# harmoniqs/DirectTrajOpt.jl

Hardware: AMD Instinct MI355X
Metric: knot-points/sec for eval_constraint_jacobian, 256-state×2000-knot bilinear (higher is better)
Workload: dtype f64; 1 GPU; configs[2]: 256-state bilinear, 4 drives, N=2000 knots per GPU (make_scaled_problem shape, Philox seed 42), callback=jacobian; state_dim=256, drives=4, knots_per_gpu=2000, knots_total=2000, parallelism=knot-range shards x1, outputs_finite=True, max_squarings=1, sweep_terms=25

## Files before the change

directtrajopt.jl_amd/csrc/dto_engine.cpp:

```cpp
#include "../../include/dto_engine.h"

#include <hip/hip_runtime.h>

#include <algorithm>
#include <chrono>
#include <cmath>
#include <cstdio>
#include <cstdlib>
#include <cstring>
#include <functional>
#include <limits>
#include <map>
#include <string>
#include <vector>

#include "dto_comm.h"
#include "dto_hostxfer.h"
#include "dto_kernels.h"

#include <memory>

using namespace dto;

namespace {
// ... 31 lines not shown

struct SweepWork {
    double* slab = nullptr;
    unsigned* arrive = nullptr;
    size_t cap = 0;
    int counters = 0;
};

struct BilHost {
    KBil k;
    SweepBuf fw{}, ad{};
    int T_alloc = 0;
    std::vector<double> g1;
    std::vector<double> n2;
    double* d_g1 = nullptr;
    double* d_n2 = nullptr;
    ChainWork chain{};
    int chain_cap = 0;
    unsigned long long* d_hump = nullptr;
    double hump_logH[4] = {0, 0, 0, 0};
    int hump_kend[4] = {0, 0, 0, 0};
    bool hump_valid = false;
    int cache_kind = 0, cache_steps = 0;
    int plan_q = 0, plan_dub = 0;
    bool p_terms = false;
    int p_steps = 0;
    int p_nblk = 0;
    SweepWork cluster_work[2];
    SweepWork gs_work[2];
    bool small = false;
    double* d_Gs = nullptr;
    bool use_basis = false;
    BasisSet basis[3]{};
    BasisSet basis_all{};
    bool pairing = false;
    double* EP = nullptr;
    double* Upair = nullptr;
    double* d_Btab = nullptr;
};

struct ConHost {
    KCon k{};
    int equality = 0;
    int64_t n_times_total = 0;
    int64_t row_off = 0;
    std::vector<int64_t> times0;
    std::vector<int32_t> comps;
    int g_dim = 1;
    bool external = false;
    bool global = false;
    int ext_slot = -1;
    std::vector<double> jac0;
    std::vector<double> hess0;
    KExtTerm xk{};
};

struct ExtObjHost {
    double weight = 1.0;
    bool global = false;
    std::vector<int32_t> comps, gcomps;
    std::vector<int64_t> times0;
    KExtTerm k{};
    int ext_slot = -1;
};

struct ExtSlot {
    dto_external_values v{nullptr, nullptr, nullptr};
// ... 74 lines not shown
    double* d_out = nullptr;
    size_t d_out_cap = 0;
    double* d_partial = nullptr;
    double* d_f = nullptr;
    double* d_bounds = nullptr;
    int32_t* d_plan = nullptr;
    double* d_jac_scratch = nullptr;
    double* d_w = nullptr;
    int64_t* d_conbase = nullptr;
    int64_t* d_crow_ptr = nullptr;
    int64_t* d_crow_col = nullptr;
    int64_t* d_crow_pos = nullptr;
    int64_t* d_con_rows = nullptr;
    double* h_pinned = nullptr;
    bool smax_pending = false;
    hipStream_t stream = nullptr;
    hipStream_t stream2 = nullptr;
    hipStream_t stream_rb = nullptr;
    hipEvent_t ev_fork = nullptr, ev_join = nullptr, ev_stats = nullptr, ev_chain = nullptr, ev_rb = nullptr, ev_zero = nullptr;

    bool reuse = false;
    double* d_Zcache = nullptr;
    int32_t* d_eq = nullptr;
    bool profiling = false;
    std::vector<ProfRec> prof;
    int64_t sweep_forms[5] = {0, 0, 0, 0, 0};
    std::vector<hipEvent_t> ev_pool;
    int last_smax = 0, last_terms = 0;
    int expm_form = 0;
    int overlap_sweep = 1;
    int sweep_form = 0;
    int chain_form = 0;
    int n_cu = 256;
    int chain_chunk = 0;
    int deterministic = 0;
    hipEvent_t ev_done = nullptr;
    bool stats_pending = false;
    int32_t* h_stats = nullptr;
    int last_form = 0;
    std::unique_ptr<Comm> comm;
    int comm_rank = -1;
    std::vector<std::pair<int64_t, int64_t>> rank_ranges;
    GatherPlan gather_plan[4];
    std::vector<Slab> cons_segments;
    std::vector<int> cons_segment_root;
    int64_t* d_ranges = nullptr;
    double* hp_slab = nullptr;
    bool hp_slab_primed = false;
    bool hp_index = false;
    KHessProduct hp{};
    int64_t hp_nnz = 0;
    int64_t* d_hp_pos = nullptr;
    double* d_hp_val = nullptr;
    double* d_hp_Z = nullptr;
    double* d_hp_mu = nullptr;
    double* d_hp_v = nullptr;
    int32_t* d_hp_eq = nullptr;
    double hp_sigma = 0.0;
    bool hp_valid = false;
    uint64_t gen = 0, hp_gen = 0;
    double hp_setup_ms = 0.0;
    double hp_bytes = 0.0;
    std::vector<void*> owned;

    ~dto_handle();
};
// ... 477 lines not shown
        enum_multisets(m1, r, cur, 0, sets[r]);
        for (size_t a = 0; a < sets[r].size(); ++a) index[r][sets[r][a]] = (int)a;
    }
    double* tmp = own(h, dalloc<double>(nn));
    std::vector<double*> S(5, nullptr);
    S[1] = const_cast<double*>(b.k.G);
    for (int r = 2; r <= 4; ++r) {
        const int cnt = (int)sets[r].size(), cntpad = ((cnt + 15) / 16) * 16;
        S[r] = own(h, dalloc<double>(nn * cntpad));
        HIP_CHECK(hipMemsetAsync(S[r], 0, nn * cntpad * sizeof(double), h->stream));
        std::vector<int32_t> idx;
        for (int a = 0; a < cnt; ++a) {
            const std::vector<int>& al = sets[r][a];
            for (int v : al) idx.push_back(v);
            int last = -1;
            for (size_t p = 0; p < al.size(); ++p) {
                const int i = al[p];
                if (i == last) continue;
                last = i;
                std::vector<int> rest = al;
                rest.erase(rest.begin() + p);
                const double* prev = S[r - 1] + (size_t)index[r - 1][rest] * nn;
                launch_bgemm_plain(h->stream, npad, 1, b.k.G + (size_t)i * nn, prev, tmp);
                launch_add(h->stream, S[r] + (size_t)a * nn, tmp, (int64_t)nn);
            }
        }
        BasisSet& bs = b.basis[r - 2];
        bs.r = r; bs.cnt = cnt; bs.cntpad = cntpad; bs.S = S[r];
        bs.idx = own(h, dupload(idx));
        const int cappad = ((cap + 127) / 128) * 128;
        bs.coef = own(h, dalloc<double>((size_t)cappad * cntpad));
    }
    {
        int cnt = 1 + m1;
        for (int r = 2; r <= 4; ++r) cnt += (int)sets[r].size();
        const int cntpad = ((cnt + 15) / 16) * 16;
        double* Sall = own(h, dalloc<double>(nn * cntpad));
        HIP_CHECK(hipMemsetAsync(Sall, 0, nn * cntpad * sizeof(double), h->stream));
        std::vector<double> eye(nn, 0.0);
        for (int i = 0; i < b.k.n; ++i) eye[(size_t)i * npad + i] = 1.0;
        HIP_CHECK(hipMemcpyAsync(Sall, eye.data(), nn * sizeof(double), hipMemcpyHostToDevice, h->stream));
        HIP_CHECK(hipStreamSynchronize(h->stream));
        std::vector<int32_t> idx;
        size_t col = 1;
        for (int q = 0; q < 4; ++q) idx.push_back(-1);
        for (int r = 1; r <= 4; ++r) {
            HIP_CHECK(hipMemcpyAsync(Sall + col * nn, S[r], nn * sets[r].size() * sizeof(double), hipMemcpyDeviceToDevice, h->stream));
            col += sets[r].size();
            for (auto& al : sets[r]) {
                for (int q = 0; q < 4; ++q) idx.push_back(q < r ? al[q] : -1);
            }
        }
        BasisSet& bs = b.basis_all;
        bs.r = 4; bs.cnt = cnt; bs.cntpad = cntpad; bs.S = Sall;
        bs.idx = own(h, dupload(idx));
        const int cappad = ((cap + 127) / 128) * 128;
        bs.coef = own(h, dalloc<double>((size_t)cappad * cntpad));
    }
    HIP_CHECK(hipStreamSynchronize(h->stream));
    b.use_basis = true;
}

void alloc_chain(dto_handle* h, BilHost& b, int cap) {
    const size_t nn = (size_t)b.k.npad * b.k.npad;
    for (int i = 0; i < 9; ++i) b.chain.W[i] = own(h, dalloc<double>(nn * cap));
    b.chain.norms = own(h, dalloc<double>((size_t)cap * 4));
    b.chain.colsum = own(h, dalloc<double>((size_t)3 * cap * b.k.npad * (b.k.npad / 64)));
    if (!b.d_hump) b.d_hump = own(h, dalloc<unsigned long long>(8));
    b.chain.coef = own(h, dalloc<double>((size_t)cap * COEF_STRIDE));
    b.chain.s = own(h, dalloc<int32_t>(cap));
    b.chain.s3 = own(h, dalloc<int32_t>(cap));
    b.chain.smax = own(h, dalloc<int32_t>(8));
    HIP_CHECK(hipMemset(b.chain.smax, 0, 8 * sizeof(int32_t)));
    b.chain.d2max = reinterpret_cast<unsigned long long*>(b.chain.smax + 2);
    b.chain_cap = cap;
}

int chunk_size(const dto_handle* h, int npad) {
    const double budget = 40e9;
    int c = (int)(budget / (9.0 * npad * (double)npad * 8.0));
    c = std::max(8, (c / 8) * 8);
    return (int)std::min<int64_t>(c, std::max<int64_t>(h->P.n_int, 1));
}

double run_chain(dto_handle* h, BilHost& b, const double* dZ, double* vals, double b1max, hipStream_t st,
                 const std::function<void(double)>& after_last_enqueue = nullptr, const std::function<void()>& in_bubble = nullptr,
                 bool nothing_waits = false) {
    const int npad = b.k.npad;
    const int64_t nint = h->P.n_int;
    double d2max = 0.0;
// ... 15 lines not shown
        }
        if (nothing_waits) {
            HIP_CHECK(hipMemcpyAsync(h->h_pinned + 28, w.smax, sizeof(int32_t), hipMemcpyDeviceToHost, st));
            h->smax_pending = true;
            h->last_form = 0;
            if (in_bubble) in_bubble();
            if (h->on_chain_chunk) h->on_chain_chunk(0, (int)nint);
            if (after_last_enqueue) after_last_enqueue(0.0);
            return 0.0;
        }
        launch_hump(st, h->P, b.k, dZ, b.d_g1, h->P.kn_lo, (int)nint, w.norms, b.d_hump);
        int32_t* hs = reinterpret_cast<int32_t*>(h->h_pinned + 2);
        HIP_CHECK(hipMemcpyAsync(hs, w.smax, 8 * sizeof(int32_t), hipMemcpyDeviceToHost, st));
        HIP_CHECK(hipMemcpyAsync(h->h_pinned + 16, b.d_hump, 8 * sizeof(unsigned long long), hipMemcpyDeviceToHost, st));
        HIP_CHECK(hipEventRecord(h->ev_chain, st));
        if (in_bubble) in_bubble();
        HIP_CHECK(hipEventSynchronize(h->ev_chain));
        h->last_form = 0;
        h->last_smax = hs[0];
        read_hump(h, b);
        {
            double dv;
            memcpy(&dv, hs + 2, sizeof(double));
            d2max = dv;
        }
        if (h->on_chain_chunk) h->on_chain_chunk(0, (int)nint);
        if (after_last_enqueue) after_last_enqueue(d2max);
        return d2max;
    }
    const double gemm_flops = 2.0 * npad * (double)npad * npad;
    h->last_smax = 0;
    const int64_t nchunk = (nint + cap - 1) / cap;
    const int per = (int)std::min<int64_t>(cap, (((nint + nchunk - 1) / nchunk) + 7) / 8 * 8);
    for (int64_t c0 = 0; c0 < nint; c0 += per) {
        const int nb = (int)std::min<int64_t>(per, nint - c0);
        const int64_t int0 = h->P.kn_lo + c0;
        ChainWork& w = b.chain;
        const int nbpad = ((nb + 127) / 128) * 128;
        if (b.use_basis) {
            launch_fill(st, w.norms, (int64_t)nb * 4, INFINITY);
            double* outs[3] = {w.W[1], w.W[2], w.W[3]};
            const size_t cs_set = (size_t)cap * npad * (npad / 64);
            double* css[3] = {w.colsum, w.colsum + cs_set, w.colsum + 2 * cs_set};
            {
                ProfScope ps(h, st, CAT_BUILD_A, 8.0 * npad * (double)npad * nb);
                launch_build_A(st, h->P, b.k, dZ, int0, nb, w.W[0]);
            }
            launch_basis_coef_multi(st, h->P, b.k, 3, b.basis, dZ, int0, nb, nbpad);
            {
                const double cols = b.basis[0].cntpad + b.basis[1].cntpad + b.basis[2].cntpad;
                ProfScope ps(h, st, CAT_BASIS_MULTI, 2.0 * npad * (double)npad * cols * nb);
                launch_basis_gemm_multi(st, npad, nb, nbpad, 3, b.basis, outs, css);
            }
            launch_norm_from_colsum_multi(st, npad, nb, 3, css, w.norms);
        } else {
            {
                ProfScope ps(h, st, CAT_BUILD_A, 8.0 * npad * (double)npad * nb);
                launch_build_A(st, h->P, b.k, dZ, int0, nb, w.W[0]);
            }
            { ProfScope ps(h, st, CAT_BGEMM, gemm_flops * nb); launch_bgemm_plain(st, npad, nb, w.W[0], w.W[0], w.W[1]); }
            { ProfScope ps(h, st, CAT_BGEMM, gemm_flops * nb); launch_bgemm_plain(st, npad, nb, w.W[0], w.W[1], w.W[2]); }
            { ProfScope ps(h, st, CAT_BGEMM, gemm_flops * nb); launch_bgemm_plain(st, npad, nb, w.W[1], w.W[1], w.W[3]); }
            launch_norm1(st, npad, nb, w);
        }
        HIP_CHECK(hipMemsetAsync(w.smax, 0, 8 * sizeof(int32_t), st));
        launch_expm_params(st, nb, s_ub, w);
        if (c0 == 0) HIP_CHECK(hipMemsetAsync(b.d_hump, 0, 8 * sizeof(unsigned long long), st));
        launch_hump(st, h->P, b.k, dZ, b.d_g1, int0, nb, w.norms, b.d_hump);
        static const int env_form = tune_int("DTO_EXPM_FORM", 0);
        int want_form = 0;
        if (env_form == 2 || env_form == 3) want_form = env_form;
        if (h->expm_form == 2 || h->expm_form == 3) want_form = h->expm_form;
        launch_expm_coef(st, nb, w, want_form);
        int32_t* hs = reinterpret_cast<int32_t*>(h->h_pinned + 2);
        static const int rb_side = tune_int("DTO_RB_STREAM", 1);
        hipEvent_t ev_s = h->ev_chain;
        auto readback = [&](hipStream_t rs) {
            HIP_CHECK(hipMemcpyAsync(hs, w.smax, 8 * sizeof(int32_t), hipMemcpyDeviceToHost, rs));
            HIP_CHECK(hipMemcpyAsync(h->h_pinned + 16, b.d_hump, 8 * sizeof(unsigned long long), hipMemcpyDeviceToHost, rs));
            HIP_CHECK(hipEventRecord(ev_s, rs));
        };
        if (rb_side) {
            HIP_CHECK(hipEventRecord(h->ev_rb, st));
            HIP_CHECK(hipStreamWaitEvent(h->stream_rb, h->ev_rb, 0));
            readback(h->stream_rb);
        }
        if (b.use_basis) {
            launch_basis_coef(st, h->P, b.k, b.basis_all, dZ, int0, nb, nbpad, w.coef);
            ProfScope ps(h, st, CAT_OTHER, 2.0 * npad * (double)npad * b.basis_all.cntpad * nb);
            launch_basis_gemm(st, npad, nb, nbpad, b.basis_all, w.W[5], nullptr);
        } else {
            launch_poly_h3(st, npad, nb, w);
        }
        if (!rb_side) readback(st);
        if (c0 == 0 && in_bubble) in_bubble();
        HIP_CHECK(hipEventSynchronize(ev_s));
        const int form = hs[6];
        if (form != 2 && form != 3) throw HipError{"propagator chain: the evaluation form did not come back from the device"};
        h->last_form = form;
        { ProfScope ps(h, st, CAT_BGEMM_HORNER, gemm_flops * nb); launch_bgemm_poly(st, npad, nb, w, 3, 5, 4, COEF_PA, 6, COEF_PB); }
        const SlabDest slab{h->P, b.k, int0, vals};
        if (form == 2) {
            ProfScope ps(h, st, CAT_BGEMM_HORNER, gemm_flops * nb);
            launch_bgemm_poly(st, npad, nb, w, 4, 6, 5, COEF_PC, -1, 0, false, &slab);
        } else {
            { ProfScope ps(h, st, CAT_BGEMM_HORNER, gemm_flops * nb); launch_bgemm_poly(st, npad, nb, w, 4, 6, 7, COEF_L, 8, COEF_R, true); }
            { ProfScope ps(h, st, CAT_BGEMM_HORNER, gemm_flops * nb); launch_bgemm_poly(st, npad, nb, w, 7, 8, 5, COEF_PC, -1, 0, false, &slab); }
        }
        const int s_max = form == 3 ? hs[4] : hs[0];
        const int s_sum = form == 3 ? hs[5] : hs[1];
        read_hump(h, b);
        {
            double dv;
            memcpy(&dv, hs + 2, sizeof(double));
            d2max = (dv == dv) ? std::max(d2max, dv) : dv;
        }
        const double sq_flops = s_max > 0 ? gemm_flops * (double)s_sum / s_max : 0.0;
        h->last_smax = std::max(h->last_smax, s_max);
        int src = 5;
        for (int it = 0; it < s_max; ++it) {
            ProfScope ps(h, st, CAT_BGEMM_SQUARE, sq_flops);
            launch_bgemm_square(st, npad, nb, w, src, src == 4 ? 5 : 4, it, h->P, b.k, int0, vals);
            src = src == 4 ? 5 : 4;
        }
        if (h->on_chain_chunk) h->on_chain_chunk(c0, nb);
    }
    if (after_last_enqueue) after_last_enqueue(d2max);
    return d2max;
}

double exact_d2(dto_handle* h, BilHost& b, const double* dZ, hipStream_t st, bool higher = false) {
    const int npad = b.k.npad;
    const int64_t nint = h->P.n_int;
    double d2max = 0.0;
    for (int64_t c0 = 0; c0 < nint; c0 += b.chain_cap) {
        const int nb = (int)std::min<int64_t>(b.chain_cap, nint - c0);
        const int64_t int0 = h->P.kn_lo + c0;
        ChainWork& w = b.chain;
        HIP_CHECK(hipMemsetAsync(w.smax, 0, 8 * sizeof(int32_t), st));
        launch_fill(st, w.norms, (int64_t)nb * 4, INFINITY);
        if (c0 == 0) HIP_CHECK(hipMemsetAsync(b.d_hump, 0, 8 * sizeof(unsigned long long), st));
        if (b.use_basis) {
            const int nbpad = ((nb + 127) / 128) * 128;
            const int nr = higher ? 3 : 1;
            for (int r = 0; r < nr; ++r) {
                double* cs = w.colsum + (size_t)r * b.chain_cap * npad * (npad / 64);
                launch_basis_coef(st, h->P, b.k, b.basis[r], dZ, int0, nb, nbpad, nullptr);
                launch_basis_gemm(st, npad, nb, nbpad, b.basis[r], nullptr, cs);
                launch_norm_from_colsum(st, npad, nb, cs, w.norms, 1 + r, higher ? nullptr : w.d2max);
            }
            if (higher) launch_beta_from_norms(st, nb, w);
        } else {
            launch_build_A(st, h->P, b.k, dZ, int0, nb, w.W[0]);
            launch_bgemm_plain(st, npad, nb, w.W[0], w.W[0], w.W[1]);
            launch_norm1_one(st, npad, nb, w, 1);
        }
        launch_hump(st, h->P, b.k, dZ, b.d_g1, int0, nb, w.norms, b.d_hump);
        int32_t* hs = reinterpret_cast<int32_t*>(h->h_pinned + 2);
// ... 2029 lines not shown
    if (std::string(name) == "sweep_form") {
        if (value != 0 && value != 1) return fail(h, "dto_set_option: sweep_form takes 0 (fused where it applies) or 1 (step per launch)");
        h->sweep_form = (int)value;
        drop_caches(h);
        return 0;
    }
    if (std::string(name) == "host_xfer") {
        if (h->plans_built) return fail(h, "dto_set_option: host_xfer must be set before the first host-pointer Jacobian / Hessian call");
        h->host_xfer = value != 0;
        return 0;
    }
    if (std::string(name) == "chain_chunk") {
        if (value < 0) return fail(h, "dto_set_option: chain_chunk must be >= 0");
        h->chain_chunk = (int)std::min<int64_t>(value, 1 << 30);
        return 0;
    }
    if (std::string(name) == "debug_bad_launch") {
#ifdef DTO_TUNING
        h->P.debug_bad_launch = value != 0;
        return 0;
#else
        return fail(h, "dto_set_option: debug_bad_launch exists in TUNING builds only (make TUNING=1: libdto_engine_t.so)");
#endif
    }
    if (std::string(name) == "host_xfer_check") {
        h->xfer_check = value != 0;
        return 0;
    }
    if (std::string(name) == "deterministic") {
        h->deterministic = value != 0;
        drop_caches(h);
        return 0;
    }
    if (std::string(name) == "expm_form") {
        if (value != 0 && value != 2 && value != 3) return fail(h, "dto_set_option: expm_form takes 0 (by cost), 2 or 3");
        h->expm_form = (int)value;
        return 0;
    }
    return fail(h, std::string("dto_set_option: unknown option ") + name);
}

int dto_profile_enable(dto_handle* h, int32_t on) {
    if (!h) return 1;
    if (on && !h->structure_only && h->ev_pool.size() < 1024) {
        (void)hipSetDevice(h->device);
        while (h->ev_pool.size() < 1024) {
            hipEvent_t e;
            if (hipEventCreate(&e) != hipSuccess) break;
            h->ev_pool.push_back(e);
        }
    }
    h->profiling = on != 0;
    return 0;
}
int dto_profile_reset(dto_handle* h) {
    if (!h) return 1;
    for (auto& r : h->prof) { h->ev_pool.push_back(r.a); h->ev_pool.push_back(r.b); }
    h->prof.clear();
    for (auto& c : h->sweep_forms) c = 0;
    return 0;
}
int dto_profile_get(dto_handle* h, const char* name, double* ms, int64_t* launches, double* flops) {
    return guarded(h, [&] {
        int cat = -1;
        bool any_gemm = false, any_basis = false;
        if (!strcmp(name, "bgemm")) any_gemm = true;
        else if (!strcmp(name, "bgemm_horner")) cat = CAT_BGEMM_HORNER;
        else if (!strcmp(name, "bgemm_square")) cat = CAT_BGEMM_SQUARE;
        else if (!strcmp(name, "bgemm_plain")) cat = CAT_BGEMM;
        else if (!strcmp(name, "chain64")) cat = CAT_CHAIN64;
        else if (!strcmp(name, "basis")) any_basis = true;
        else if (!strcmp(name, "basis_k")) cat = CAT_OTHER;
        else if (!strcmp(name, "basis_multi")) cat = CAT_BASIS_MULTI;
        else if (!strcmp(name, "zero_fill")) cat = CAT_ZERO;
        else if (!strcmp(name, "build_A")) cat = CAT_BUILD_A;
        else if (!strcmp(name, "assembly")) cat = CAT_ASSEMBLY;
        else if (!strcmp(name, "expmv")) cat = CAT_SWEEP;
        else if (!strcmp(name, "expmv_adjoint")) cat = CAT_SWEEP_ADJOINT;
        else if (!strcmp(name, "hess_product")) cat = CAT_HESS_PRODUCT;
        else if (!strcmp(name, "hess_product_setup")) {
            if (ms) *ms = h->hp_setup_ms;
            if (launches) *launches = 0;
            if (flops) *flops = h->hp_bytes;
            return;
        }
        else if (!strncmp(name, "sweep_", 6)) {
            static const char* const forms[5] = {"sweep_gs", "sweep_fused", "sweep_s64", "sweep_cluster", "sweep_step"};
            int f = 0;
            while (f < 5 && strcmp(name, forms[f])) ++f;
            if (f == 5) throw HipError{"dto_profile_get: unknown name"};
            if (ms) *ms = 0.0;
            if (launches) *launches = h->sweep_forms[f];
            if (flops) *flops = 0.0;
            return;
        }
        else if (strcmp(name, "all")) throw HipError{"dto_profile_get: unknown name"};
        double tot = 0, fl = 0;
        int64_t n = 0;
        for (auto& r : h->prof) {
            if (any_gemm && r.cat != CAT_BGEMM && r.cat != CAT_BGEMM_HORNER && r.cat != CAT_BGEMM_SQUARE && r.cat != CAT_CHAIN64) continue;
            if (any_basis && r.cat != CAT_OTHER && r.cat != CAT_BASIS_MULTI) continue;
            if (!any_gemm && !any_basis && cat >= 0 && r.cat != cat) continue;
            HIP_CHECK(hipEventSynchronize(r.b));
            float t = 0;
            HIP_CHECK(hipEventElapsedTime(&t, r.a, r.b));
            tot += t; fl += r.flops; ++n;
        }
        if (ms) *ms = tot;
        if (launches) *launches = n;
        if (flops) *flops = fl;
    });
}
int dto_last_stats(const dto_handle* h, int32_t* max_squarings, int32_t* expmv_terms) {
    if (!h) return 1;
    dto_handle* hm = const_cast<dto_handle*>(h);
    int rc = guarded(hm, [&] { HIP_CHECK(hipDeviceSynchronize()); }, G_BLOCKING);
    if (max_squarings) *max_squarings = h->last_smax;
    if (expmv_terms) *expmv_terms = h->last_terms;
// ... 5 lines not shown
```

directtrajopt.jl_amd/csrc/dto_kernels.h:

```cpp
#pragma once
#include <hip/hip_runtime.h>
#include <stdint.h>

#include <cstdlib>

namespace dto {

inline int tune_int(const char* name, int dflt) {
#ifdef DTO_TUNING
    const char* e = getenv(name);
    return e ? atoi(e) : dflt;
#else
    (void)name;
    return dflt;
#endif
}
inline double tune_double(const char* name, double dflt) {
#ifdef DTO_TUNING
    const char* e = getenv(name);
    return e ? atof(e) : dflt;
#else
    (void)name;
    return dflt;
#endif
// ... 84 lines not shown
    else
        colstart = tri + (kn - 1) * (z * z + tri) + (int64_t)b * z + (int64_t)b * (b + 1) / 2 + z;
    return colstart + a - P.hess_lo;
}

struct TypeDesc {
    int32_t n_extra;
    int32_t gen[2];
    int32_t src[2];
    double mult[2];
};

struct SweepTypes {
    int32_t T;
    TypeDesc t[MAX_TYPES];
};

struct ChainWork {
    double* W[9];
    double* norms;
    double* colsum;
    double* coef;
    int32_t* s;
    int32_t* s3;
    int32_t* smax;
    unsigned long long* d2max;
};

void launch_build_A(hipStream_t st, const KProb& P, const KBil& B, const double* dZ, int64_t int0, int nb, double* A);
void launch_bgemm_plain(hipStream_t st, int npad, int nb, const double* A, const double* Bm, double* C);
void launch_norm1(hipStream_t st, int npad, int nb, const ChainWork& w);
void launch_norm1_one(hipStream_t st, int npad, int nb, const ChainWork& w, int which);
void launch_expm_params(hipStream_t st, int nb, int s_cap, const ChainWork& w);
void launch_expm_coef(hipStream_t st, int nb, const ChainWork& w, int form);
void launch_poly_h3(hipStream_t st, int npad, int nb, const ChainWork& w);
struct SlabDest {
    KProb P;
    KBil B;
    int64_t int0;
    double* vals;
};
void launch_bgemm_poly(hipStream_t st, int npad, int nb, const ChainWork& w, int srcA, int srcB, int dst, int coef_base,
                       int dst2, int coef_base2, bool with_srcA = false, const SlabDest* slab = nullptr);
void launch_bgemm_square(hipStream_t st, int npad, int nb, const ChainWork& w, int src, int dst, int it,
                         const KProb& P, const KBil& B, int64_t int0, double* vals);

hipError_t chain64_prepare();
hipError_t launch_chain64(hipStream_t st, const KProb& P, const KBil& B, const double* dZ, double* vals, double* norms, int32_t* smax,
                          unsigned long long* d2max, int32_t* sk, int s_cap, int force_form, int n_cu);

struct SweepBuf {
    int32_t npad, Kpad, TN;
    double* Z[2];
    double* S;
    double* GY;
    double* W;
    double* scaleA;
    double* scaleU;
    double* scaleE;
    unsigned long long* termnorm;
    unsigned long long* sumnorm;
    int32_t* active;
    int32_t* stats;
    double* Zt;
    int32_t dcap, T_alloc;
    int32_t* nterms;
    int32_t* nterms_p;
// ... 163 lines not shown
};
void launch_jac_spmv(hipStream_t st, const KProb& P, const KIntegTable& T, const int64_t* conbase, const int64_t* con_rows,
                     const double* vals, const double* w, double* y, int transpose, int64_t global_cols = 0);
void launch_jac_rowgather(hipStream_t st, const KProb& P, const KIntegTable& T, int64_t n_con_rows, const int64_t* rptr, const int64_t* rcol,
                          const int64_t* rpos, int64_t n_dyn, const double* vals, const double* w, double* y);
void launch_add(hipStream_t st, double* dst, const double* src, int64_t n);
void launch_bits_equal(hipStream_t st, const double* a, const double* b, int64_t n, int32_t* flag);

struct KHessProduct {
    const int64_t* start;
    const int32_t* len;
    const int32_t* col;
    const double* val;
    const int32_t* rows;
    int64_t row0[4], blk0[4];
    int32_t cls_g[3];
    int32_t n_cls;
};
void launch_hess_gather(hipStream_t st, const double* slab, const int64_t* pos, int64_t n, double* val);
void launch_hess_spmv(hipStream_t st, const KHessProduct& p, const double* v, double* y);

struct BasisSet {
    int32_t r, cnt, cntpad;
    const double* S;
    const int32_t* idx;
    double* coef;
};
void launch_basis_coef(hipStream_t st, const KProb& P, const KBil& B, const BasisSet& bs, const double* dZ,
                       int64_t int0, int nb, int nbpad, const double* taylor);
void launch_jac_zero(hipStream_t st, const KProb& P, const KBil& B, double* vals);
void launch_basis_gemm(hipStream_t st, int npad, int nb, int nbpad, const BasisSet& bs, double* out, double* colsum);
void launch_basis_gemm_multi(hipStream_t st, int npad, int nb, int nbpad, int nsets, const BasisSet* bs, double* const* out,
                             double* const* colsum);
void launch_basis_coef_multi(hipStream_t st, const KProb& P, const KBil& B, int nsets, const BasisSet* bs, const double* dZ,
                             int64_t int0, int nb, int nbpad);
void launch_norm_from_colsum_multi(hipStream_t st, int npad, int nb, int nsets, double* const* colsum, double* norms);
void launch_beta_from_norms(hipStream_t st, int nb, const ChainWork& w);
void launch_hump(hipStream_t st, const KProb& P, const KBil& B, const double* dZ, const double* g1, int64_t int0, int nb,
                 const double* norms, unsigned long long* out);
void launch_norm_from_colsum(hipStream_t st, int npad, int nb, const double* colsum, double* norms, int which,
                             unsigned long long* d2max = nullptr);
void launch_norm_bounds(hipStream_t st, const KProb& P, const KBil& B, const double* dZ, const double* g1,
                        const double* n2, unsigned long long* out2);

}
```

directtrajopt.jl_amd/csrc/dto_kernels.hip:

```cpp
#include "dto_gemm.hip.h"
#include "dto_gemm_ring.hip.h"
#include "dto_kernels.h"
#include "dto_hostxfer.h"

#include <cstdlib>
#include <string>
#include <vector>

namespace dto {

__device__ __forceinline__ unsigned long long dbits(double v) { return (unsigned long long)__double_as_longlong(fabs(v)); }
__device__ __forceinline__ double bits_to_d(unsigned long long b) { return __longlong_as_double((long long)b); }

__device__ __forceinline__ void hess_add(const KProb& P, double* H, int64_t kn, int a, int b, double v);

static inline dim3 blk(const KProb& P, int threads) { return dim3(P.debug_bad_launch ? 4096 : threads); }

__device__ __forceinline__ double wave_sum(double v) {
#pragma unroll
    for (int o = 32; o > 0; o >>= 1) v += __shfl_xor(v, o, 64);
    return v;
}
__device__ __forceinline__ double wave_max(double v) {
#pragma unroll
// ... 205 lines not shown
};
template <class Cfg>
__global__ void __launch_bounds__(Cfg::THREADS, 2) k_basis_gemm_multi(int npad, int nb, BasisMulti M) {
    __shared__ __attribute__((aligned(1024))) double smem[Cfg::SMEM_DOUBLES];
    const int which = blockIdx.x % M.nsets, tile = blockIdx.x / M.nsets;
    BasisSet bs = M.bs[0];
    double* out = M.out[0];
    double* colsum = M.colsum[0];
#pragma unroll
    for (int q = 1; q < 4; ++q)
        if (q == which) { bs = M.bs[q]; out = M.out[q]; colsum = M.colsum[q]; }
    const int64_t nn = (int64_t)npad * npad;
    const int row_tiles = (int)(nn / Cfg::TM);
    const int rt = tile % row_tiles, ct = tile / row_tiles;
    GemmAccS<Cfg> acc;
    acc.zero();
    basis_accumulate<Cfg>(acc, bs, nn, rt, ct, smem);
    basis_epilogue<Cfg>(acc, npad, nb, rt, ct, out, colsum);
}
void launch_basis_gemm_multi(hipStream_t st, int npad, int nb, int nbpad, int nsets, const BasisSet* bs, double* const* out,
                             double* const* colsum) {
    const int64_t nn = (int64_t)npad * npad;
    BasisMulti M{};
    M.nsets = nsets;
    for (int q = 0; q < nsets; ++q) { M.bs[q] = bs[q]; M.out[q] = out[q]; M.colsum[q] = colsum[q]; }
    const dim3 grid((unsigned)((nn / 128) * (nbpad / 128) * nsets));
    static const int core = tune_int("DTO_BASIS_CORE", 1);
    if (core == 1) {
        using C = GemmShapeP<128, 128, 2, 4>;
        hipLaunchKernelGGL((k_basis_gemm_multi<C>), grid, dim3(C::THREADS), 0, st, npad, nb, M);
    } else {
        using C = GemmShape<128, 128, 2, 4, 16>;
        hipLaunchKernelGGL((k_basis_gemm_multi<C>), grid, dim3(C::THREADS), 0, st, npad, nb, M);
    }
}
__global__ void k_basis_coef_multi(KProb P, KBil B, BasisMulti M, const double* __restrict__ Z, int64_t int0, int nb) {
    const int b = blockIdx.x;
    BasisSet bs = M.bs[0];
#pragma unroll
    for (int q = 1; q < 4; ++q)
        if (q == (int)blockIdx.y) bs = M.bs[q];
    double* c = bs.coef + (int64_t)b * bs.cntpad;
    if (b >= nb) {
        for (int a = threadIdx.x; a < bs.cntpad; a += blockDim.x) c[a] = 0.0;
        return;
    }
    const double* zk = Z + (int0 + b) * P.z;
    const double dt = zk[P.dt_idx];
    for (int a = threadIdx.x; a < bs.cntpad; a += blockDim.x) {
        double v = 0.0;
        if (a < bs.cnt) {
            v = 1.0;
            for (int i = 0; i < bs.r; ++i) {
                const int g = bs.idx[a * bs.r + i];
                v *= dt;
                if (g > 0) v *= zk[B.u_off + g - 1];
            }
        }
        c[a] = v;
    }
}
void launch_basis_coef_multi(hipStream_t st, const KProb& P, const KBil& B, int nsets, const BasisSet* bs, const double* dZ,
                             int64_t int0, int nb, int nbpad) {
    BasisMulti M{};
    M.nsets = nsets;
    for (int q = 0; q < nsets; ++q) M.bs[q] = bs[q];
// ... 711 lines not shown
    for (int k = 1; k <= 160; ++k) {
        const double v = fmin(fmin(b0 + lN[1], b1 + lN[2]), fmin(b2 + lN[3], b3 + lN[4]));
        b3 = b2; b2 = b1; b1 = b0; b0 = v;
        lfact += logk[k];
        const double lt = v - lfact;
        logH = fmax(logH, lt);
        if (lt >= -43.75) kend = k;
        else if (logk[k] > rate) break;
    }
    if (bad) { logH = __longlong_as_double(0x7ff8000000000000ll); kend = 160; }
    unsigned long long hb = dbits(logH), kb = (unsigned long long)kend;
#pragma unroll
    for (int o = 4; o < 64; o <<= 1) {
        const unsigned long long h2 = __shfl_xor(hb, o, 64), k2 = __shfl_xor(kb, o, 64);
        hb = h2 > hb ? h2 : hb;
        kb = k2 > kb ? k2 : kb;
    }
    if ((threadIdx.x & 63) < 4) {
        atomicMax(&out[q - 1], hb);
        atomicMax(&out[4 + q - 1], kb);
    }
}
void launch_hump(hipStream_t st, const KProb& P, const KBil& B, const double* dZ, const double* g1, int64_t int0, int nb,
                 const double* norms, unsigned long long* out) {
    hipLaunchKernelGGL(k_hump, dim3((4 * nb + 255) / 256), dim3(256), 0, st, P, B, dZ, g1, int0, nb, norms, out);
}
void launch_norm1(hipStream_t st, int npad, int nb, const ChainWork& w) {
    hipLaunchKernelGGL(k_norm1, dim3(nb, 4), dim3(256), 0, st, npad, w, -1);
}
void launch_norm1_one(hipStream_t st, int npad, int nb, const ChainWork& w, int which) {
    hipLaunchKernelGGL(k_norm1, dim3(nb, 1), dim3(256), 0, st, npad, w, which);
}

__global__ void k_expm_params(int nb, int s_cap, ChainWork w) {
    const int b = blockIdx.x * blockDim.x + threadIdx.x;
    if (b >= nb) return;
    const double n1 = w.norms[b * 4 + 0];
    const double d2v = sqrt(w.norms[b * 4 + 1]);
    const double d3v = cbrt(w.norms[b * 4 + 2]);
    const double d4v = sqrt(sqrt(w.norms[b * 4 + 3]));
    double alpha = fmin(n1, fmin(fmax(d2v, d3v), fmax(d3v, d4v)));
    int s = 0;
    if (alpha > THETA_16) {
        s = (int)ceil(log2(alpha / THETA_16));
        if (s < 1) s = 1;
    }
    if (s > s_cap) s = s_cap;
    if (!(alpha == alpha)) s = 1;
    w.s[b] = s;
    atomicMax(&w.smax[0], s);
    atomicAdd(&w.smax[1], s);
    int s3 = 0;
    if (alpha > THETA_3P) {
        s3 = (int)ceil(log2(alpha / THETA_3P));
        if (s3 < 1) s3 = 1;
    }
    if (s3 > s_cap) s3 = s_cap;
    if (!(alpha == alpha)) s3 = 1;
    w.s3[b] = s3;
    atomicMax(&w.smax[4], s3);
    atomicAdd(&w.smax[5], s3);
    double beta = fmin(d2v, fmax(d3v, d4v));
    if (!(d2v == d2v) || !(d3v == d3v) || !(d4v == d4v)) beta = __longlong_as_double(0x7ff8000000000000ll);
    atomicMax(w.d2max, dbits(beta));
}
__global__ void k_expm_coef(int nb, ChainWork w, int form) {
    const int b = blockIdx.x * blockDim.x + threadIdx.x;
    if (form == 0) form = 2 * ((int64_t)w.smax[1] - (int64_t)w.smax[5]) > 3 * (int64_t)nb ? 3 : 2;
    if (b == 0) w.smax[6] = form;
    if (b >= nb) return;
    int s = w.s[b];
    if (form == 3) { s = w.s3[b]; w.s[b] = s; }
    const double sigma = ldexp(1.0, -s);
    double* cf = w.coef + (int64_t)b * COEF_STRIDE;
    double sp = 1.0;
    const double s4 = (sigma * sigma) * (sigma * sigma);
    for (int i = 0; i <= 4; ++i) {
        if (form == 3) {
            cf[COEF_PC + i] = EXPM3_E[i] * sp;
            cf[COEF_PA + i] = EXPM3_A[i] * sp;
            cf[COEF_PB + i] = EXPM3_B[i] * sp;
            cf[COEF_K + i] = EXPM3_K[i] * sp * s4;
            cf[COEF_L + i] = (EXPM3_C[i] - EXPM3_AL * EXPM3_A[i]) * sp;
            cf[COEF_R + i] = (EXPM3_D[i] - EXPM3_BE * EXPM3_A[i]) * sp;
        } else {
            cf[COEF_PC + i] = EXPM2_C[i] * sp;
            cf[COEF_PA + i] = EXPM2_A[i] * sp;
            cf[COEF_PB + i] = EXPM2_B[i] * sp;
            cf[COEF_K + i] = EXPM2_K[i] * sp * s4;
        }
        sp *= sigma;
    }
    cf[COEF_L + 5] = EXPM3_AL;
    cf[COEF_R + 5] = EXPM3_BE;
}
void launch_expm_coef(hipStream_t st, int nb, const ChainWork& w, int form) {
    hipLaunchKernelGGL(k_expm_coef, dim3((nb + 63) / 64), dim3(64), 0, st, nb, w, form);
}
void launch_expm_params(hipStream_t st, int nb, int s_cap, const ChainWork& w) {
    hipLaunchKernelGGL(k_expm_params, dim3((nb + 63) / 64), dim3(64), 0, st, nb, s_cap, w);
}

__global__ void __launch_bounds__(256) k_poly_h3(int npad, ChainWork w) {
    const int b = blockIdx.y;
    const int64_t nn = (int64_t)npad * npad;
    const double* cf = w.coef + (int64_t)b * COEF_STRIDE + COEF_K;
    const double c0 = cf[0], c1 = cf[1], c2 = cf[2], c3 = cf[3], c4 = cf[4];
    const double* A1 = w.W[0] + b * nn;
    const double* A2 = w.W[1] + b * nn;
    const double* A3 = w.W[2] + b * nn;
    const double* A4 = w.W[3] + b * nn;
    double* H = w.W[5] + b * nn;
    for (int64_t i = (int64_t)blockIdx.x * 256 + threadIdx.x; i < nn; i += (int64_t)gridDim.x * 256) {
        double v = c1 * A1[i] + c2 * A2[i] + c3 * A3[i] + c4 * A4[i];
        if (i % npad == i / npad) v += c0;
        H[i] = v;
    }
}
void launch_poly_h3(hipStream_t st, int npad, int nb, const ChainWork& w) {
    int gx = (int)(((int64_t)npad * npad + 255) / 256);
    if (gx > 64) gx = 64;
    hipLaunchKernelGGL(k_poly_h3, dim3(gx, nb), dim3(256), 0, st, npad, w);
}


__global__ void __launch_bounds__(256) k_sweep_init(KProb P, KBil B, SweepBuf w, int T, const double* __restrict__ Z,
                                                     const double* __restrict__ mu, int src_kind, double inv_q) {
    const int k = blockIdx.x;
    const bool live = k < P.n_int;
    const int64_t kn = P.kn_lo + k;
// ... 1194 lines not shown
```

Baseline: 190,300 knot-points/s.

## Carry scaling plan across calls to fuse Taylor-K build into basis GEMM

Replaces the separate all-basis coefficient+GEMM pass that built the expm polynomial K with a fused kernel. The fused kernel accumulates the degree-1..4 basis products and applies per-knot scaling coefficients, reusing the s values saved from the previous call when the plan key matches. Only column blocks whose scaling or form changed since the last call are recomputed by a repair pass. The Horner GEMM launch is also moved ahead of the host sync on the form readback. This adds persistent state across calls and relies on the scaling decisions staying stable between evaluations.

```diff
diff --git a/directtrajopt.jl_amd/csrc/dto_engine.cpp b/directtrajopt.jl_amd/csrc/dto_engine.cpp
--- a/directtrajopt.jl_amd/csrc/dto_engine.cpp
+++ b/directtrajopt.jl_amd/csrc/dto_engine.cpp
@@ -87,7 +87,12 @@
     double* d_Gs = nullptr;
     bool use_basis = false;
     BasisSet basis[3]{};
-    BasisSet basis_all{};
+    BasisSet basis1{};
+    int32_t* s_prev = nullptr;
+    int32_t* form_prev = nullptr;
+    int32_t* rep_list = nullptr;
+    bool plan_valid = false;
+    int64_t plan_key[4] = {-1, -1, -1, -1};
     bool pairing = false;
     double* EP = nullptr;
     double* Upair = nullptr;
@@ -228,6 +233,8 @@
     int sweep_form = 0;
     int chain_form = 0;
     int n_cu = 256;
+    int carry_plan = 1;
+    int64_t k_repair = 0;
     int chain_chunk = 0;
     int deterministic = 0;
     hipEvent_t ev_done = nullptr;
@@ -771,30 +778,23 @@
         bs.coef = own(h, dalloc<double>((size_t)cappad * cntpad));
     }
     {
-        int cnt = 1 + m1;
-        for (int r = 2; r <= 4; ++r) cnt += (int)sets[r].size();
-        const int cntpad = ((cnt + 15) / 16) * 16;
-        double* Sall = own(h, dalloc<double>(nn * cntpad));
-        HIP_CHECK(hipMemsetAsync(Sall, 0, nn * cntpad * sizeof(double), h->stream));
-        std::vector<double> eye(nn, 0.0);
-        for (int i = 0; i < b.k.n; ++i) eye[(size_t)i * npad + i] = 1.0;
-        HIP_CHECK(hipMemcpyAsync(Sall, eye.data(), nn * sizeof(double), hipMemcpyHostToDevice, h->stream));
-        HIP_CHECK(hipStreamSynchronize(h->stream));
-        std::vector<int32_t> idx;
-        size_t col = 1;
-        for (int q = 0; q < 4; ++q) idx.push_back(-1);
-        for (int r = 1; r <= 4; ++r) {
-            HIP_CHECK(hipMemcpyAsync(Sall + col * nn, S[r], nn * sets[r].size() * sizeof(double), hipMemcpyDeviceToDevice, h->stream));
-            col += sets[r].size();
-            for (auto& al : sets[r]) {
-                for (int q = 0; q < 4; ++q) idx.push_back(q < r ? al[q] : -1);
-            }
-        }
-        BasisSet& bs = b.basis_all;
-        bs.r = 4; bs.cnt = cnt; bs.cntpad = cntpad; bs.S = Sall;
+        const int cntpad = 16;
+        if (m1 > cntpad) throw HipError{"build_basis: more than 16 generators"};
+        double* S1 = own(h, dalloc<double>(nn * cntpad));
+        HIP_CHECK(hipMemsetAsync(S1, 0, nn * cntpad * sizeof(double), h->stream));
+        HIP_CHECK(hipMemcpyAsync(S1, b.k.G, nn * m1 * sizeof(double), hipMemcpyDeviceToDevice, h->stream));
+        std::vector<int32_t> idx(m1);
+        for (int i = 0; i < m1; ++i) idx[i] = i;
+        BasisSet& bs = b.basis1;
+        bs.r = 1; bs.cnt = m1; bs.cntpad = cntpad; bs.S = S1;
         bs.idx = own(h, dupload(idx));
         const int cappad = ((cap + 127) / 128) * 128;
         bs.coef = own(h, dalloc<double>((size_t)cappad * cntpad));
+        const int64_t nint = std::max<int64_t>(h->P.n_int, 1);
+        b.s_prev = own(h, dalloc<int32_t>(nint));
+        b.form_prev = own(h, dalloc<int32_t>(nint / 8 + 2));
+        b.rep_list = own(h, dalloc<int32_t>(cappad / 128));
+        b.plan_valid = false;
     }
     HIP_CHECK(hipStreamSynchronize(h->stream));
     b.use_basis = true;
@@ -876,6 +876,10 @@
     h->last_smax = 0;
     const int64_t nchunk = (nint + cap - 1) / cap;
     const int per = (int)std::min<int64_t>(cap, (((nint + nchunk - 1) / nchunk) + 7) / 8 * 8);
+    static const int env_form0 = tune_int("DTO_EXPM_FORM", 0);
+    const int64_t plan_key[4] = {h->P.kn_lo, nint, per, h->expm_form == 2 || h->expm_form == 3 ? h->expm_form : env_form0};
+    const bool carried = b.use_basis && h->carry_plan && b.plan_valid && !memcmp(plan_key, b.plan_key, sizeof(plan_key));
+    b.plan_valid = false;
     for (int64_t c0 = 0; c0 < nint; c0 += per) {
         const int nb = (int)std::min<int64_t>(per, nint - c0);
         const int64_t int0 = h->P.kn_lo + c0;
@@ -890,9 +894,14 @@
                 ProfScope ps(h, st, CAT_BUILD_A, 8.0 * npad * (double)npad * nb);
                 launch_build_A(st, h->P, b.k, dZ, int0, nb, w.W[0]);
             }
-            launch_basis_coef_multi(st, h->P, b.k, 3, b.basis, dZ, int0, nb, nbpad);
-            {
-                const double cols = b.basis[0].cntpad + b.basis[1].cntpad + b.basis[2].cntpad;
+            const BasisSet sets4[4] = {b.basis[0], b.basis[1], b.basis[2], b.basis1};
+            launch_basis_coef_multi(st, h->P, b.k, 4, sets4, dZ, int0, nb, nbpad);
+            const double cols = b.basis[0].cntpad + b.basis[1].cntpad + b.basis[2].cntpad;
+            if (carried) {
+                ProfScope ps(h, st, CAT_BASIS_MULTI, 2.0 * npad * (double)npad * (cols + b.basis1.cntpad) * nb);
+                launch_basis_gemm_k(st, npad, nb, nbpad, b.basis, b.basis1, outs, css, w.W[5], b.s_prev + c0, b.form_prev + c0 / per,
+                                    b.k.n, false, nullptr, nullptr);
+            } else {
                 ProfScope ps(h, st, CAT_BASIS_MULTI, 2.0 * npad * (double)npad * cols * nb);
                 launch_basis_gemm_multi(st, npad, nb, nbpad, 3, b.basis, outs, css);
             }
@@ -915,7 +924,8 @@
         int want_form = 0;
         if (env_form == 2 || env_form == 3) want_form = env_form;
         if (h->expm_form == 2 || h->expm_form == 3) want_form = h->expm_form;
-        launch_expm_coef(st, nb, w, want_form);
+        if (b.use_basis) launch_expm_coef(st, nb, w, want_form, b.s_prev + c0, b.form_prev + c0 / per, b.rep_list, carried);
+        else launch_expm_coef(st, nb, w, want_form);
         int32_t* hs = reinterpret_cast<int32_t*>(h->h_pinned + 2);
         static const int rb_side = tune_int("DTO_RB_STREAM", 1);
         hipEvent_t ev_s = h->ev_chain;
@@ -929,20 +939,32 @@
             HIP_CHECK(hipStreamWaitEvent(h->stream_rb, h->ev_rb, 0));
             readback(h->stream_rb);
         }
+        const double cols_k = b.use_basis ? b.basis[0].cntpad + b.basis[1].cntpad + b.basis[2].cntpad + b.basis1.cntpad : 0.0;
         if (b.use_basis) {
-            launch_basis_coef(st, h->P, b.k, b.basis_all, dZ, int0, nb, nbpad, w.coef);
-            ProfScope ps(h, st, CAT_OTHER, 2.0 * npad * (double)npad * b.basis_all.cntpad * nb);
-            launch_basis_gemm(st, npad, nb, nbpad, b.basis_all, w.W[5], nullptr);
+            if (!carried) {
+                ProfScope ps(h, st, CAT_OTHER, 2.0 * npad * (double)npad * cols_k * nbpad);
+                launch_basis_gemm_k(st, npad, nb, nbpad, b.basis, b.basis1, nullptr, nullptr, w.W[5], w.s, w.smax + 6, b.k.n, true,
+                                    nullptr, nullptr);
+                h->k_repair += nbpad / 128;
+            } else {
+                launch_basis_gemm_k(st, npad, nb, nbpad, b.basis, b.basis1, nullptr, nullptr, w.W[5], w.s, w.smax + 6, b.k.n, true,
+                                    b.rep_list, w.smax + 7);
+            }
         } else {
             launch_poly_h3(st, npad, nb, w);
         }
         if (!rb_side) readback(st);
         if (c0 == 0 && in_bubble) in_bubble();
+        { ProfScope ps(h, st, CAT_BGEMM_HORNER, gemm_flops * nb); launch_bgemm_poly(st, npad, nb, w, 3, 5, 4, COEF_PA, 6, COEF_PB); }
         HIP_CHECK(hipEventSynchronize(ev_s));
         const int form = hs[6];
         if (form != 2 && form != 3) throw HipError{"propagator chain: the evaluation form did not come back from the device"};
         h->last_form = form;
-        { ProfScope ps(h, st, CAT_BGEMM_HORNER, gemm_flops * nb); launch_bgemm_poly(st, npad, nb, w, 3, 5, 4, COEF_PA, 6, COEF_PB); }
+        if (carried) {
+            const int nrep = hs[7];
+            if (nrep < 0 || nrep > nbpad / 128) throw HipError{"propagator chain: bad repair count from the device"};
+            h->k_repair += nrep;
+        }
         const SlabDest slab{h->P, b.k, int0, vals};
         if (form == 2) {
             ProfScope ps(h, st, CAT_BGEMM_HORNER, gemm_flops * nb);
@@ -968,6 +990,10 @@
             src = src == 4 ? 5 : 4;
         }
         if (h->on_chain_chunk) h->on_chain_chunk(c0, nb);
+    }
+    if (b.use_basis) {
+        memcpy(b.plan_key, plan_key, sizeof(plan_key));
+        b.plan_valid = true;
     }
     if (after_last_enqueue) after_last_enqueue(d2max);
     return d2max;
@@ -3063,6 +3089,11 @@
         drop_caches(h);
         return 0;
     }
+    if (std::string(name) == "carry_plan") {
+        if (value != 0 && value != 1) return fail(h, "dto_set_option: carry_plan takes 0 or 1");
+        h->carry_plan = (int)value;
+        return 0;
+    }
     if (std::string(name) == "expm_form") {
         if (value != 0 && value != 2 && value != 3) return fail(h, "dto_set_option: expm_form takes 0 (by cost), 2 or 3");
         h->expm_form = (int)value;
@@ -3089,6 +3120,7 @@
     for (auto& r : h->prof) { h->ev_pool.push_back(r.a); h->ev_pool.push_back(r.b); }
     h->prof.clear();
     for (auto& c : h->sweep_forms) c = 0;
+    h->k_repair = 0;
     return 0;
 }
 int dto_profile_get(dto_handle* h, const char* name, double* ms, int64_t* launches, double* flops) {
@@ -3115,6 +3147,12 @@
             if (flops) *flops = h->hp_bytes;
             return;
         }
+        else if (!strcmp(name, "k_repair")) {
+            if (ms) *ms = 0.0;
+            if (launches) *launches = h->k_repair;
+            if (flops) *flops = 0.0;
+            return;
+        }
         else if (!strncmp(name, "sweep_", 6)) {
             static const char* const forms[5] = {"sweep_gs", "sweep_fused", "sweep_s64", "sweep_cluster", "sweep_step"};
             int f = 0;
diff --git a/directtrajopt.jl_amd/csrc/dto_kernels.h b/directtrajopt.jl_amd/csrc/dto_kernels.h
--- a/directtrajopt.jl_amd/csrc/dto_kernels.h
+++ b/directtrajopt.jl_amd/csrc/dto_kernels.h
@@ -140,7 +140,8 @@
 void launch_norm1(hipStream_t st, int npad, int nb, const ChainWork& w);
 void launch_norm1_one(hipStream_t st, int npad, int nb, const ChainWork& w, int which);
 void launch_expm_params(hipStream_t st, int nb, int s_cap, const ChainWork& w);
-void launch_expm_coef(hipStream_t st, int nb, const ChainWork& w, int form);
+void launch_expm_coef(hipStream_t st, int nb, const ChainWork& w, int form, int32_t* s_prev = nullptr, int32_t* form_prev = nullptr,
+                      int32_t* rep_list = nullptr, bool check = false);
 void launch_poly_h3(hipStream_t st, int npad, int nb, const ChainWork& w);
 struct SlabDest {
     KProb P;
@@ -370,6 +371,9 @@
 void launch_basis_gemm(hipStream_t st, int npad, int nb, int nbpad, const BasisSet& bs, double* out, double* colsum);
 void launch_basis_gemm_multi(hipStream_t st, int npad, int nb, int nbpad, int nsets, const BasisSet* bs, double* const* out,
                              double* const* colsum);
+void launch_basis_gemm_k(hipStream_t st, int npad, int nb, int nbpad, const BasisSet* bs, const BasisSet& bs1, double* const* out,
+                         double* const* colsum, double* outK, const int32_t* s, const int32_t* form, int n, bool k_only,
+                         const int32_t* blocks, const int32_t* nblocks);
 void launch_basis_coef_multi(hipStream_t st, const KProb& P, const KBil& B, int nsets, const BasisSet* bs, const double* dZ,
                              int64_t int0, int nb, int nbpad);
 void launch_norm_from_colsum_multi(hipStream_t st, int npad, int nb, int nsets, double* const* colsum, double* norms);
diff --git a/directtrajopt.jl_amd/csrc/dto_kernels.hip b/directtrajopt.jl_amd/csrc/dto_kernels.hip
--- a/directtrajopt.jl_amd/csrc/dto_kernels.hip
+++ b/directtrajopt.jl_amd/csrc/dto_kernels.hip
@@ -261,6 +261,116 @@
     } else {
         using C = GemmShape<128, 128, 2, 4, 16>;
         hipLaunchKernelGGL((k_basis_gemm_multi<C>), grid, dim3(C::THREADS), 0, st, npad, nb, M);
+    }
+}
+struct BasisKPlan {
+    double* outK;
+    const int32_t* s;
+    const int32_t* form;
+    const int32_t* blocks;
+    const int32_t* nblocks;
+    int n;
+};
+template <class Cfg>
+__device__ __forceinline__ int basis_k_row(int row0, int ti) {
+    if constexpr (Cfg::PAIRED) return row0 + 32 * (ti / 2) + (ti & 1);
+    else return row0 + 16 * ti;
+}
+template <class Cfg>
+__device__ __forceinline__ void basis_k_add(GemmAccS<Cfg>& kacc, const GemmAccS<Cfg>& acc, const int (&sk)[Cfg::NT][4], int form, int deg) {
+    double k2 = EXPM2_K[1], k3 = EXPM3_K[1];
+#pragma unroll
+    for (int d = 2; d <= 4; ++d)
+        if (d == deg) { k2 = EXPM2_K[d]; k3 = EXPM3_K[d]; }
+    const double kd = form == 3 ? k3 : k2;
+#pragma unroll
+    for (int tj = 0; tj < Cfg::NT; ++tj)
+#pragma unroll
+        for (int r = 0; r < 4; ++r) {
+            const double c = ldexp(kd, -sk[tj][r] * (4 + deg));
+#pragma unroll
+            for (int ti = 0; ti < Cfg::MT; ++ti) kacc.v[ti][tj][r] = fma(c, acc.v[ti][tj][r], kacc.v[ti][tj][r]);
+        }
+}
+template <class Cfg, bool KONLY>
+__global__ void __launch_bounds__(Cfg::THREADS, 2) k_basis_gemm_k(int npad, int nb, BasisMulti M, BasisKPlan Kp) {
+    __shared__ __attribute__((aligned(1024))) double smem[Cfg::SMEM_DOUBLES];
+    const int64_t nn = (int64_t)npad * npad;
+    const int row_tiles = (int)(nn / Cfg::TM);
+    const int rt = blockIdx.x % row_tiles;
+    int ct = blockIdx.x / row_tiles;
+    if (KONLY && Kp.blocks) {
+        if (ct >= Kp.nblocks[0]) return;
+        ct = Kp.blocks[ct];
+    }
+    int row0, col0;
+    if constexpr (Cfg::PAIRED) { GemmCoordP<Cfg> co; row0 = rt * Cfg::TM + co.row_base; col0 = ct * Cfg::TN + co.col_base; }
+    else { GemmCoordS<Cfg> co; row0 = rt * Cfg::TM + co.row_base; col0 = ct * Cfg::TN + co.col_base; }
+    const int form = Kp.form[0];
+    int sk[Cfg::NT][4];
+#pragma unroll
+    for (int tj = 0; tj < Cfg::NT; ++tj)
+#pragma unroll
+        for (int r = 0; r < 4; ++r) {
+            const int col = col0 + 16 * tj + 4 * r;
+            sk[tj][r] = col < nb ? Kp.s[col] : 0;
+        }
+    GemmAccS<Cfg> kacc, acc;
+    kacc.zero();
+#pragma unroll 1
+    for (int it = 0; it < 4; ++it) {
+        const int q = it < 3 ? 2 - it : 3;
+        acc.zero();
+        basis_accumulate<Cfg>(acc, M.bs[q], nn, rt, ct, smem);
+        if constexpr (!KONLY)
+            if (q < 3) basis_epilogue<Cfg>(acc, npad, nb, rt, ct, M.out[q], M.colsum[q]);
+        basis_k_add<Cfg>(kacc, acc, sk, form, q < 3 ? q + 2 : 1);
+    }
+    const double k0 = form == 3 ? EXPM3_K[0] : EXPM2_K[0];
+#pragma unroll
+    for (int tj = 0; tj < Cfg::NT; ++tj)
+#pragma unroll
+        for (int r = 0; r < 4; ++r) {
+            const int col = col0 + 16 * tj + 4 * r;
+            if (col >= nb) continue;
+            const double c0 = ldexp(k0, -4 * sk[tj][r]);
+            double* dst = Kp.outK + (int64_t)col * nn;
+#pragma unroll
+            for (int ti = 0; ti < Cfg::MT; ++ti) {
+                const int row = basis_k_row<Cfg>(row0, ti);
+                if (row % (npad + 1) == 0 && row / (npad + 1) < Kp.n) kacc.v[ti][tj][r] += c0;
+            }
+            if constexpr (Cfg::PAIRED) {
+#pragma unroll
+                for (int p = 0; p < Cfg::MT / 2; ++p) {
+                    const d2 v = {kacc.v[2 * p][tj][r], kacc.v[2 * p + 1][tj][r]};
+                    __builtin_nontemporal_store(v, reinterpret_cast<d2*>(&dst[row0 + 32 * p]));
+                }
+            } else {
+#pragma unroll
+                for (int ti = 0; ti < Cfg::MT; ++ti) __builtin_nontemporal_store(kacc.v[ti][tj][r], &dst[row0 + 16 * ti]);
+            }
+        }
+}
+void launch_basis_gemm_k(hipStream_t st, int npad, int nb, int nbpad, const BasisSet* bs, const BasisSet& bs1, double* const* out,
+                         double* const* colsum, double* outK, const int32_t* s, const int32_t* form, int n, bool k_only,
+                         const int32_t* blocks, const int32_t* nblocks) {
+    const int64_t nn = (int64_t)npad * npad;
+    BasisMulti M{};
+    M.nsets = 4;
+    for (int q = 0; q < 3; ++q) { M.bs[q] = bs[q]; M.out[q] = k_only ? nullptr : out[q]; M.colsum[q] = k_only ? nullptr : colsum[q]; }
+    M.bs[3] = bs1;
+    BasisKPlan Kp{outK, s, form, blocks, nblocks, n};
+    const dim3 grid((unsigned)((nn / 128) * (nbpad / 128)));
+    static const int core = tune_int("DTO_BASIS_CORE", 1);
+    if (core == 1) {
+        using C = GemmShapeP<128, 128, 2, 4>;
+        if (k_only) hipLaunchKernelGGL((k_basis_gemm_k<C, true>), grid, dim3(C::THREADS), 0, st, npad, nb, M, Kp);
+        else hipLaunchKernelGGL((k_basis_gemm_k<C, false>), grid, dim3(C::THREADS), 0, st, npad, nb, M, Kp);
+    } else {
+        using C = GemmShape<128, 128, 2, 4, 16>;
+        if (k_only) hipLaunchKernelGGL((k_basis_gemm_k<C, true>), grid, dim3(C::THREADS), 0, st, npad, nb, M, Kp);
+        else hipLaunchKernelGGL((k_basis_gemm_k<C, false>), grid, dim3(C::THREADS), 0, st, npad, nb, M, Kp);
     }
 }
 __global__ void k_basis_coef_multi(KProb P, KBil B, BasisMulti M, const double* __restrict__ Z, int64_t int0, int nb) {
@@ -1038,6 +1148,8 @@
     hipLaunchKernelGGL(k_norm1, dim3(nb, 1), dim3(256), 0, st, npad, w, which);
 }
 
+__global__ void k_set_i32(int32_t* dst, const int32_t* src) { *dst = *src; }
+
 __global__ void k_expm_params(int nb, int s_cap, ChainWork w) {
     const int b = blockIdx.x * blockDim.x + threadIdx.x;
     if (b >= nb) return;
@@ -1070,13 +1182,23 @@
     if (!(d2v == d2v) || !(d3v == d3v) || !(d4v == d4v)) beta = __longlong_as_double(0x7ff8000000000000ll);
     atomicMax(w.d2max, dbits(beta));
 }
-__global__ void k_expm_coef(int nb, ChainWork w, int form) {
+__global__ void __launch_bounds__(128) k_expm_coef(int nb, ChainWork w, int form, int32_t* s_prev, int32_t* form_prev, int32_t* rep_list,
+                                                   int check) {
     const int b = blockIdx.x * blockDim.x + threadIdx.x;
     if (form == 0) form = 2 * ((int64_t)w.smax[1] - (int64_t)w.smax[5]) > 3 * (int64_t)nb ? 3 : 2;
     if (b == 0) w.smax[6] = form;
+    int s = 0;
+    if (b < nb) {
+        s = w.s[b];
+        if (form == 3) { s = w.s3[b]; w.s[b] = s; }
+    }
+    if (s_prev) {
+        const int stale = check && b < nb && (form_prev[0] != form || s_prev[b] != s);
+        const int any = __syncthreads_or(stale);
+        if (b < nb) s_prev[b] = s;
+        if (threadIdx.x == 0 && any) rep_list[atomicAdd(&w.smax[7], 1)] = blockIdx.x;
+    }
     if (b >= nb) return;
-    int s = w.s[b];
-    if (form == 3) { s = w.s3[b]; w.s[b] = s; }
     const double sigma = ldexp(1.0, -s);
     double* cf = w.coef + (int64_t)b * COEF_STRIDE;
     double sp = 1.0;
@@ -1100,8 +1222,10 @@
     cf[COEF_L + 5] = EXPM3_AL;
     cf[COEF_R + 5] = EXPM3_BE;
 }
-void launch_expm_coef(hipStream_t st, int nb, const ChainWork& w, int form) {
-    hipLaunchKernelGGL(k_expm_coef, dim3((nb + 63) / 64), dim3(64), 0, st, nb, w, form);
+void launch_expm_coef(hipStream_t st, int nb, const ChainWork& w, int form, int32_t* s_prev, int32_t* form_prev, int32_t* rep_list,
+                      bool check) {
+    hipLaunchKernelGGL(k_expm_coef, dim3((nb + 127) / 128), dim3(128), 0, st, nb, w, form, s_prev, form_prev, rep_list, check ? 1 : 0);
+    if (form_prev) hipLaunchKernelGGL(k_set_i32, dim3(1), dim3(1), 0, st, form_prev, w.smax + 6);
 }
 void launch_expm_params(hipStream_t st, int nb, int s_cap, const ChainWork& w) {
     hipLaunchKernelGGL(k_expm_params, dim3((nb + 63) / 64), dim3(64), 0, st, nb, s_cap, w);
```

Result: no change. 190,900 knot-points/s, median of 6 (+0.3%).
